# ydchen0806/CLC

Hardware: AMD Instinct MI355X
Metric: images/sec fwd+bwd @256x256 bs8; bpp+PSNR parity vs ref (higher is better)
Workload: dtype f32; 1 GPU; CLC N=64 lambda=0.0067 MSE, 256x256 bs8/GPU, n_refs=1: fwd + RD loss + bwd + clip_grad_norm + AdamW + aux step (configs[1]); global_batch=8, parallelism=dp1, ranks_seen=1, collective=none, hip_graph=True

## Files before the change

clc_amd/csrc/common.h:

```cpp
#pragma once
#include <hip/hip_runtime.h>
#include <stdarg.h>
#include <stdio.h>
#include "../../include/clc_hip.h"

typedef float f32x2 __attribute__((ext_vector_type(2)));
typedef float f32x4 __attribute__((ext_vector_type(4)));
typedef float f32x16 __attribute__((ext_vector_type(16)));

void clc_set_error(const char* fmt, ...);

enum {  CLC_TUNE_WGRAD_STREAMK = 1,
       CLC_TUNE_SPLITK_PIX = 4 , CLC_TUNE_SPLITK_MAXC = 5 ,
       CLC_TUNE_SPLITK_PF = 6 ,
       CLC_TUNE_1X1_TILE = 7 ,
       CLC_TUNE_XCD_MAP = 8 ,
       CLC_TUNE_WGRAD_DMA = 9 ,
       CLC_TUNE_REG_EPI = 10 ,
       CLC_TUNE_DGRAD_SPLITK = 11 ,
       CLC_TUNE_P1X1 = 13 ,
       CLC_TUNE_BF16 = 14 ,
       CLC_TUNE_TILE256 = 15 ,
       CLC_TUNE_ATTN_4B = 16 ,
       CLC_TUNE_HEAVY128 = 17 ,
       CLC_TUNE_ATTN_SPLIT = 18 ,
       CLC_TUNE_N16 = 20 ,
       CLC_TUNE_LIN = 21 ,
       CLC_TUNE_HALO = 22 ,
       CLC_TUNE_WINO = 23 ,
       CLC_TUNE_SPLIT = 24 ,
       CLC_TUNE_COUNT = 25 };
extern int clc_tuning[CLC_TUNE_COUNT];
int clc_conv_halo_launch(const void* conv_params, const float* wpk, hipStream_t st);
int clc_conv_wino_launch(const void* conv_params, const float* u, hipStream_t st);
int clc_conv5_launch(const clc_conv_desc* d, hipStream_t st);
size_t clc_conv5_wgrad_workspace_bytes(const clc_wgrad_desc* d);
int clc_conv5_wgrad_launch(const clc_wgrad_desc* d, hipStream_t st);
int clc_lin_launch(const float* x, int ldx, const float* w, const float* bias, const float* res, int ldr, float res_scale, float* y, int ldy, long M, int Cin,
                   int Cout, hipStream_t st);

#define CLC_CHECK(cond, ...)            \
  do {                                  \
    if (!(cond)) {                      \
      clc_set_error(__VA_ARGS__);       \
      return -1;                        \
    }                                   \
  } while (0)

#define CLC_LAUNCH_CHECK()                                              \
  do {                                                                  \
    hipError_t e_ = hipGetLastError();                                  \
    if (e_ != hipSuccess) {                                             \
      clc_set_error("%s:%d launch failed: %s", __FILE__, __LINE__, hipGetErrorString(e_)); \
      return -2;                                                        \
    }                                                                   \
  } while (0)

struct PerDeviceOnce {
  bool done[32] = {};
  bool first() {
    int d = 0;
    if (hipGetDevice(&d) != hipSuccess || d < 0 || d >= 32) return true;
    if (done[d]) return false;
    done[d] = true;
    return true;
  }
};
// ... 130 lines not shown
```

clc_amd/csrc/conv_igemm.hip:

```cpp
#include "common.h"
#ifndef CLC_PF32
#define CLC_PF32 3
#endif

namespace {
#include "conv_common.h"
template <int BM, int BN, int WM, int WN, bool TR>
__global__ __launch_bounds__(64 * WM * WN, (64 * WM * WN) >= 512 ? 4 : ((64 * WM * WN) >= 256 ? 2 : 4))
void conv_igemm_kernel(const ConvParams p) {
  constexpr int NT = 64 * WM * WN;
  constexpr int TM = BM / WM / 32, TN = BN / WN / 32;
  constexpr int A_P = BM * 8 / NT, B_P = BN * 8 / NT;
  static_assert(TM >= 1 && TN >= 1 && A_P * NT == BM * 8 && B_P * NT == BN * 8, "tile");
  extern __shared__ __attribute__((aligned(16))) float smem[];
  float* As = smem;
  float* Bs = smem + 2 * BM * LD;

  const int tid = threadIdx.x, lane = tid & 63, wave = tid >> 6;
  const int wm = wave / WN, wn = wave % WN;
  const int m0 = blockIdx.x * BM, n0 = blockIdx.y * BN;
  const int cls = blockIdx.z, ph = cls >> 1, pw = cls & 1;
  const bool half = p.transposed && p.stride == 2;
  const int DH = half ? p.OH / 2 : p.OH, DW = half ? p.OW / 2 : p.OW;
  const TapGrid tg = make_taps(p, ph, pw);
// ... 1020 lines not shown
extern "C" size_t clc_conv2d_workspace_bytes(const clc_conv_desc* d) {
  if (!d || d->ks == 5) return 0;
  ConvParams p;
  int classes = 1;
  if (fill_params(d, p, classes) < 0) return 0;
  const bool vec_ok = (d->Cin % 4 == 0) && (d->ldx % 4 == 0) && aligned16(d->x) && aligned16(d->w);
  if (!vec_ok || d->Cout < 64) return 0;
  const int img_pix = (d->transposed && d->stride == 2) ? (d->OH / 2) * (d->OW / 2) : d->OH * d->OW;
  if (img_pix > 1024) return 0;
  const int k = conv_ksplit(p, classes);
  return k > 1 ? (size_t)k * classes * p.M * p.Cout * sizeof(float) : 0;
}

extern "C" int clc_conv2d(const clc_conv_desc* d, clc_stream_t stream) {
  hipStream_t st = (hipStream_t)stream;
  if (d && d->ks == 5) return clc_conv5_launch(d, st);
  ConvParams p;
  int classes = 1;
  if (fill_params(d, p, classes) < 0) return -1;
  const bool vec_ok = (d->Cin % 4 == 0) && (d->ldx % 4 == 0) && aligned16(d->x) && aligned16(d->w);
  if (!vec_ok) {
    CLC_CHECK(!d->transposed && !d->xs, "clc_conv2d: unaligned/small-Cin path has no transposed / fused-activation mode (Cin=%d ldx=%d)", d->Cin, d->ldx);
    const int cgroups = (d->Cout + 3) / 4;
    const long total = (long)p.M * cgroups;
    hipLaunchKernelGGL(conv_direct_small_kernel, dim3((unsigned)((total + 255) / 256)), dim3(256), 0, st, p);
    CLC_LAUNCH_CHECK();
    return 1;
  }
  const int img_pix = (d->transposed && d->stride == 2) ? (d->OH / 2) * (d->OW / 2) : d->OH * d->OW;
  const int C = d->Cout;
  const int splitk_pix = clc_tuning[CLC_TUNE_SPLITK_PIX] > 0 ? clc_tuning[CLC_TUNE_SPLITK_PIX] : 256;
  const bool small_map = img_pix <= 256 || (img_pix <= splitk_pix && C <= clc_tuning[CLC_TUNE_SPLITK_MAXC]);
  if (small_map) {
    if (heavy128_split(p, classes) > 1) {
      use_split(p, d, classes);
      if (p.ksplit > 1) return launch<128, 128, 4, 2>(p, classes, st);
    }
    if (img_pix <= 256 && d->transposed && d->ks * d->ks * p.kc_tiles >= 60 && C >= 128 &&
        (long)((p.M + 63) / 64) * ((C + 63) / 64) * classes >= 128) {
      use_split(p, d, classes);
      return launch<64, 64, 2, 2>(p, classes, st);
    }
    const long wg32 = (long)((p.M + 31) / 32) * ((C + 31) / 32) * classes;
    if (C > 32 && wg32 > 256) return launch_splitk<64>(p, classes, st);
    return launch_splitk<32>(p, classes, st);
  }
  p.bf16 = clc_tuning[CLC_TUNE_BF16] != 0 && img_pix > 256;
  if ((clc_tuning[CLC_TUNE_WINO] & (d->transposed ? 2 : 1)) && d->w_wino && d->ks == 3 && d->stride == 1 && classes == 1) {
    const int v = clc_conv_wino_launch(&p, d->w_wino, st);
    if (v) return v;
  }
  if (clc_tuning[CLC_TUNE_HALO] && d->w_packed && d->ks == 3 && d->stride == 1 && classes == 1) {
    const int v = clc_conv_halo_launch(&p, d->w_packed, st);
    if (v) return v;
  }
  if (img_pix <= 1024) {
    if (C >= 64) {
      use_split(p, d, classes);
      return launch<64, 64, 2, 2>(p, classes, st);
    }
    return launch<64, 32, 2, 1>(p, classes, st);
  }
  if (clc_tuning[CLC_TUNE_LIN] && d->ks == 1 && d->stride == 1 && classes == 1 && vec_ok && !p.shuffle && !p.group_rows && !p.xs && p.in_op == CLC_IN_NONE &&
      p.act == CLC_ACT_NONE && p.norm == CLC_NORM_NONE && !p.y_pre && !p.res_gate && !p.out_gate && p.ldw == p.Cin && p.vec_epi && !p.bf16) {
    const int v = clc_lin_launch(p.x, p.ldx, p.w, p.bias, p.res, p.ldr, p.res_scale, p.y, p.ldy, p.M, p.Cin, p.Cout, st);
    if (v) { CLC_LAUNCH_CHECK(); return v; }
  }
  if (d->ks == 1 && C > 32 && vec_ok) {
    const int v = launch_p1x1(p, classes, st);
    if (v) return v;
  }
  if (clc_tuning[CLC_TUNE_1X1_TILE] && d->ks == 1 && p.kc_tiles <= clc_tuning[CLC_TUNE_1X1_TILE] && C > 32) return launch<128, 64, 4, 2>(p, classes, st);
  if (C % 128 == 0 || C >= 384) return launch<128, 128, 4, 2>(p, classes, st);
  if (clc_tuning[CLC_TUNE_TILE256] && d->ks == 3 && C > 32 && C <= 64 && p.M >= 256 * 512 && (!p.group_rows || p.group_rows % 256 == 0))
    return launch<256, 64, 4, 2>(p, classes, st);
  if (C > 32) return launch<128, 64, 4, 2>(p, classes, st);
  if (C <= 16 && vec_ok) {
    const int v = launch_n16(p, classes, st);
    if (v) return v;
  }
  if (clc_tuning[CLC_TUNE_TILE256] && d->ks == 3 && p.M % 128 == 0 && p.M >= 128 * 512) return launch<128, 32, 2, 1>(p, classes, st);
  return launch<64, 32, 2, 1>(p, classes, st);
// ... 10 lines not shown
```

clc_amd/csrc/conv_wino.hip:

```cpp
#include "common.h"

namespace {
#include "conv_common.h"

constexpr int TH = 8, TW = 16, HW = TW + 2, HPIX = (TH + 2) * HW;
constexpr int HALO_FLOATS = HPIX * 128;
constexpr int PIECES = HPIX / 2;

struct WinoParams {
  ConvParams c;
  const float* u;
  int items, ntn, ncg;
  unsigned u_bytes;
};

#ifndef WINO_AB
#define WINO_AB 0
#endif
#if WINO_AB & 32
__device__ unsigned long long wino_dbg[32];
#define WINO_STAMP(k) do { if (blockIdx.x == 0 && tid == 0 && it == i0 + 1) wino_dbg[k] = __builtin_amdgcn_s_memtime(); } while (0)
#else
#define WINO_STAMP(k) do { } while (0)
#endif
#define MFMA(a, b, c) __builtin_amdgcn_mfma_f32_32x32x2f32((a), (b), (c), 0, 0, 0)

constexpr int VB_FLOATS = 16 * 32 * 16;

template <bool SHUF>
__global__ __launch_bounds__(512, 1) void conv_wino_kernel(const WinoParams wp) {
  const ConvParams& p = wp.c;
  extern __shared__ __attribute__((aligned(16))) float smem[];
  float* halo = smem;
  float* bias_s = smem + HALO_FLOATS + 2 * VB_FLOATS;
  float* VV = smem + HALO_FLOATS;
  const int tid = threadIdx.x, lane = tid & 63, wave = tid >> 6;
  const int li = lane & 31, h = lane >> 5;
  const int tiles_w = p.W / TW, tiles_h = p.H / TH;
  const int KCT = wp.ncg * 4;
  const int NC16 = wp.ncg * 8;
  const int i0 = (int)((long)wp.items * blockIdx.x / gridDim.x), i1 = (int)((long)wp.items * (blockIdx.x + 1) / gridDim.x);
  const __amdgpu_buffer_rsrc_t xr = __builtin_amdgcn_make_buffer_rsrc(const_cast<float*>(p.x), 0, p.x_bytes, 0x00020000);
  const __amdgpu_buffer_rsrc_t ur = __builtin_amdgcn_make_buffer_rsrc(const_cast<float*>(wp.u), 0, wp.u_bytes, 0x00020000);
  const int q = tid & 3, t = (tid >> 2) & 31, part = tid >> 7;
  const int ty = t >> 3, tx = t & 7;
  const int wi = wave >> 1, nh = wave & 1;
// ... 204 lines not shown
        } else {
#pragma unroll 1
          for (int a = 0; a < 2; ++a)
#pragma unroll 1
            for (int e = 0; e < 4; ++e) {
              epilogue_store(p, a ? y[1][0][e] : y[0][0][e], bv[e], mrow0 + a * p.OW, co + e, p.OH, p.OW, 0, 0);
              epilogue_store(p, a ? y[1][1][e] : y[0][1][e], bv[e], mrow0 + a * p.OW + 1, co + e, p.OH, p.OW, 0, 0);
            }
        }
      }
      WINO_STAMP(15 + 3 * rd);
    }
  }
}

constexpr int HALO2_FLOATS = HPIX * 64;
constexpr int S2_FLOATS = 16 * 32 * 32;
constexpr int PIECES2 = HPIX / 4;
static_assert(HALO2_FLOATS <= S2_FLOATS, "the halo lies inside the output round's image");
__device__ __forceinline__ int wino64_swz(int hy, int hx) { return ((hx >> 1) & 3) | (((hy >> 1) & 3) << 2); }
__device__ __forceinline__ float add1(float a, float b) { float r; asm("v_add_f32 %0, %1, %2" : "=v"(r) : "v"(a), "v"(b)); return r; }
__device__ __forceinline__ float sub1(float a, float b) { float r; asm("v_sub_f32 %0, %1, %2" : "=v"(r) : "v"(a), "v"(b)); return r; }
__device__ __forceinline__ float fma1(float s, float b, float a) { float r; asm("v_fma_f32 %0, %1, %2, %3" : "=v"(r) : "s"(s), "v"(b), "v"(a)); return r; }

template <bool SHUF>
__global__ __launch_bounds__(256, 2) void conv_wino64_kernel(const WinoParams wp) {
  const ConvParams& p = wp.c;
  extern __shared__ __attribute__((aligned(16))) float smem[];
  float* halo = smem;
  float* S = smem;
  const int tid = threadIdx.x, lane = tid & 63, wave = __builtin_amdgcn_readfirstlane(tid >> 6);
  const int li = lane & 31, h = lane >> 5;
  const int tiles_w = p.W / TW, tiles_h = p.H / TH;
  const int KCT = wp.ncg * 2;
  const int NC16 = wp.ncg * 4;
  const int i0 = (int)((long)wp.items * blockIdx.x / gridDim.x), i1 = (int)((long)wp.items * (blockIdx.x + 1) / gridDim.x);
  const __amdgpu_buffer_rsrc_t xr = __builtin_amdgcn_make_buffer_rsrc(const_cast<float*>(p.x), 0, p.x_bytes, 0x00020000);
  const __amdgpu_buffer_rsrc_t ur = __builtin_amdgcn_make_buffer_rsrc(const_cast<float*>(wp.u), 0, wp.u_bytes, 0x00020000);
  const int ty = li >> 3, tx = li & 7;
  const int qo = tid & 15;
  const bool lean = epilogue_is_lean(p);
  const int ra = wave == 0 ? 0 : (wave == 2 ? 2 : 1), rb = wave == 0 ? 2 : (wave == 1 ? 2 : (wave == 2 ? 1 : 3));
  const float sg = wave == 1 ? 1.f : -1.f;
  int pa[2][2];
#pragma unroll
  for (int rr = 0; rr < 2; ++rr)
#pragma unroll
    for (int ch = 0; ch < 2; ++ch) {
      const int hy = 2 * ty + (rr ? rb : ra);
      pa[rr][ch] = (hy * HW + 2 * tx) * 256 + ((h ^ wino64_swz(hy, 2 * tx + 2 * ch)) << 4);
    }
  const char* hb = reinterpret_cast<const char*>(halo);
  auto read_row = [&](f32x4 (&d)[4], int rr, int kx) {
#pragma unroll
    for (int c = 0; c < 4; ++c) d[c] = *reinterpret_cast<const f32x4*>(hb + ((pa[rr][c >> 1] ^ kx) + c * 256));
  };
  const unsigned b_lane = (unsigned)lane * 16u;

  for (int it = i0; it < i1; ++it) {
    const int pt = it / wp.ntn, nt = it - pt * wp.ntn;
    const int txx = pt % tiles_w, t2 = pt / tiles_w, tyy = t2 % tiles_h, n = t2 / tiles_h;
    const int oy0 = tyy * TH, ox0 = txx * TW;
    f32x16 acc[4][2];
#pragma unroll
    for (int s = 0; s < 4; ++s)
#pragma unroll
      for (int nb = 0; nb < 2; ++nb)
#pragma unroll
        for (int r = 0; r < 16; ++r) acc[s][nb][r] = 0.f;
    f32x4 bq[4][2];
    auto load_b = [&](int s, int c16, int t8) {
      const int kcg = c16 >> 1, t8g = 2 * (c16 & 1) + t8;
#pragma unroll
      for (int nb = 0; nb < 2; ++nb)
        bq[s][nb] = buf_load4(ur, b_lane + (unsigned)((((((nt >> 1) * 16 + 4 * wave + s) * KCT + kcg) * 4 + 2 * (nt & 1) + nb) * 4 + t8g)) * 1024u);
    };
#pragma unroll
    for (int s = 0; s < 4; ++s) load_b(s, 0, 0);
    WINO_STAMP(0);

    for (int cg = 0; cg < wp.ncg; ++cg) {
      if (cg) __syncthreads();
      {
        const int org = ((n * p.H + oy0 - 1) * p.W + ox0 - 1) * p.ldx + cg * 64;
        int hy = 0, hx = 4 * wave + (lane >> 4);
#pragma unroll 1
        for (int pc = wave; pc < PIECES2; pc += 4) {
          const int iy = oy0 - 1 + hy, ix = ox0 - 1 + hx;
          const bool ok = (unsigned)iy < (unsigned)p.H && (unsigned)ix < (unsigned)p.W;
          const int c = (lane & 15) ^ wino64_swz(hy, hx);
          dma16(xr, halo + pc * 256, ok ? (unsigned)(org + (hy * p.W + hx) * p.ldx + c * 4) * 4u : kOOB);
          hx += 16;
          if (hx >= HW) { hx -= HW; ++hy; }
        }
        asm volatile("s_waitcnt vmcnt(0)" ::: "memory");
      }
      __syncthreads();
      WINO_STAMP(1);
      f32x4 aq[2][4];
      f32x4 da[4], db[4];
      auto rows_T = [&]() {
#pragma unroll
        for (int c = 0; c < 4; ++c)
#pragma unroll
          for (int e = 0; e < 4; ++e) da[c][e] = fma1(sg, db[c][e], da[c][e]);
      };
      auto cols_B = [&](f32x4 (&v)[4]) {
#pragma unroll
        for (int e = 0; e < 4; ++e) {
          v[0][e] = sub1(da[0][e], da[2][e]);
          v[1][e] = add1(da[1][e], da[2][e]);
          v[2][e] = sub1(da[2][e], da[1][e]);
          v[3][e] = sub1(da[1][e], da[3][e]);
        }
      };
      read_row(da, 0, 0);
      read_row(db, 1, 0);
      rows_T();
      cols_B(aq[0]);
      WINO_STAMP(2);
#pragma unroll 1
      for (int kc = 0; kc < 4; ++kc) {
        if (cg == 0) WINO_STAMP(3 + kc);
        const int c16 = cg * 4 + kc;
#pragma unroll
        for (int t8 = 0; t8 < 2; ++t8) {
          const int kxn = t8 == 0 ? (4 * kc + 2) << 4 : (4 * ((kc + 1) & 3)) << 4;
          const int c16n = t8 == 0 ? c16 : (c16 + 1 < NC16 ? c16 + 1 : 0);
#pragma unroll
          for (int s = 0; s < 4; ++s) {
            if (s == 0) read_row(da, 0, kxn);
            else if (s == 1) read_row(db, 1, kxn);
            else if (s == 2) rows_T();
            else cols_B(aq[t8 ^ 1]);
            __builtin_amdgcn_sched_barrier(0);
#pragma unroll
            for (int ss = 0; ss < 4; ++ss)
#pragma unroll
              for (int nb = 0; nb < 2; ++nb) acc[s][nb] = MFMA(aq[t8][s][ss], bq[s][nb][ss], acc[s][nb]);
            load_b(s, c16n, t8 ^ 1);
            __builtin_amdgcn_sched_barrier(0);
          }
        }
      }
    }
    WINO_STAMP(11);
    {
      const int co = nt * 64 + (qo >> 3) * 32 + (qo & 7) * 4;
      const f32x4 bv = epilogue_bias4(p.bias, co);
      __syncthreads();
      WINO_STAMP(13);
#pragma unroll
      for (int b = 0; b < 2; ++b) {
        float* dst = S + ((wave * 2 + b) * 32) * 64;
#pragma unroll
// ... 100 lines not shown
    f32x4 u[4];
    u[0] = tt[i][0];
    u[1] = 0.5f * ((tt[i][0] + tt[i][1]) + tt[i][2]);
    u[2] = 0.5f * ((tt[i][0] - tt[i][1]) + tt[i][2]);
    u[3] = tt[i][2];
#pragma unroll
    for (int j = 0; j < 4; ++j) {
      const size_t idx = ((((((size_t)nt * 16 + (i * 4 + j)) * KCT + kcg) * 4 + nb) * 4 + t8) * 64 + lane);
      *reinterpret_cast<f32x4*>(out + idx * 4) = u[j];
    }
  }
}
__global__ void filter_wino_kernel(const float* __restrict__ w, float* __restrict__ out, int N, int K, int flip) {
  const long e = (long)blockIdx.x * blockDim.x + threadIdx.x;
  if (e >= (long)N * K / 4) return;
  wino_u_one(w, out, e, K, flip);
}
__global__ void filter_wino_batched_kernel(const clc_wino_entry* __restrict__ table, int n_entries) {
  int lo = 0, hi = n_entries - 1;
  const int b = blockIdx.x;
  while (lo < hi) {
    const int mid = (lo + hi + 1) >> 1;
    if (table[mid].block_begin <= b) lo = mid; else hi = mid - 1;
  }
  const clc_wino_entry en = table[lo];
  const long e = (long)(b - en.block_begin) * blockDim.x + threadIdx.x;
  if (e >= (long)en.N * en.K / 4) return;
  wino_u_one(en.w, en.out, e, en.K, en.flip);
}

}

extern "C" int clc_filter_wino(const float* w, float* out, int N, int K, int flip, clc_stream_t stream) {
  CLC_CHECK(w && out && N > 0 && N % 64 == 0 && K > 0 && K % 64 == 0 && aligned16(w) && aligned16(out),
            "clc_filter_wino: rows and channels must be positive multiples of 64, pointers 16-B aligned (got N=%d K=%d)", N, K);
  const long total = (long)N * K / 4;
  hipLaunchKernelGGL(filter_wino_kernel, dim3((unsigned)((total + 255) / 256)), dim3(256), 0, (hipStream_t)stream, w, out, N, K, flip);
  CLC_LAUNCH_CHECK();
  return 0;
}
extern "C" int clc_filter_wino_batched(const clc_wino_entry* table_dev, int n_entries, int total_blocks, clc_stream_t stream) {
  CLC_CHECK(table_dev && n_entries > 0 && total_blocks > 0, "clc_filter_wino_batched: bad args");
  hipLaunchKernelGGL(filter_wino_batched_kernel, dim3(total_blocks), dim3(256), 0, (hipStream_t)stream, table_dev, n_entries);
  CLC_LAUNCH_CHECK();
  return 0;
}

int clc_conv_wino_launch(const void* conv_params, const float* u, hipStream_t st) {
  const ConvParams& p = *reinterpret_cast<const ConvParams*>(conv_params);
  if (!u || p.ks != 3 || p.stride != 1 || p.pad != 1 || p.Cin % 64 || p.Cin > 1024 || p.Cout % 64 || p.H % TH || p.W % TW || p.OH != p.H || p.OW != p.W) return 0;
  if (p.xs || p.in_op != CLC_IN_NONE || p.group_rows || p.bf16 || p.ksplit > 1 || p.ldx % 4 || !aligned16(p.x) || !aligned16(u)) return 0;
  const bool shuf = p.shuffle != 0;
  if (!shuf && !p.vec_epi) return 0;
  const size_t ub = (size_t)((p.Cout + 127) / 128 * 128) * 16 * p.Cin * 4;
  if (ub >= (1ull << 31)) return 0;
  const int mode = clc_tuning[CLC_TUNE_WINO];
  const int ptiles = p.N * (p.H / TH) * (p.W / TW);
  const bool can128 = p.Cin % 128 == 0 && p.Cout % 128 == 0 && !(mode & 8);
  const bool wide = can128 && ptiles * (p.Cout / 128) >= 192;
  if (!wide && (!(mode & 4) || ptiles * (p.Cout / 64) < 128)) return 0;
  const int nw = wide ? 128 : 64;
  WinoParams wp;
  wp.c = p;
  wp.u = u;
  wp.ntn = p.Cout / nw;
  wp.ncg = p.Cin / nw;
  wp.items = ptiles * wp.ntn;
  wp.u_bytes = (unsigned)ub;
  static PerDeviceOnce once[2];
  const int k = shuf ? 1 : 0;
  if (wide) {
    const int grid = wp.items < 256 ? wp.items : 256;
    const int lds = (HALO_FLOATS + 2 * VB_FLOATS + 128) * 4;
    static PerDeviceOnce oncep[2];
    if (shuf) {
      if (oncep[0].first()) (void)hipFuncSetAttribute(reinterpret_cast<const void*>(conv_wino_kernel<true>), hipFuncAttributeMaxDynamicSharedMemorySize, lds);
      hipLaunchKernelGGL(conv_wino_kernel<true>, dim3(grid), dim3(512), lds, st, wp);
    } else {
      if (oncep[1].first()) (void)hipFuncSetAttribute(reinterpret_cast<const void*>(conv_wino_kernel<false>), hipFuncAttributeMaxDynamicSharedMemorySize, lds);
      hipLaunchKernelGGL(conv_wino_kernel<false>, dim3(grid), dim3(512), lds, st, wp);
    }
  } else {
    const int grid = wp.items < 512 ? wp.items : 512;
    const int lds = S2_FLOATS * 4;
    if (shuf) {
      if (once[k].first()) (void)hipFuncSetAttribute(reinterpret_cast<const void*>(conv_wino64_kernel<true>), hipFuncAttributeMaxDynamicSharedMemorySize, lds);
      hipLaunchKernelGGL(conv_wino64_kernel<true>, dim3(grid), dim3(256), lds, st, wp);
    } else {
      if (once[k].first()) (void)hipFuncSetAttribute(reinterpret_cast<const void*>(conv_wino64_kernel<false>), hipFuncAttributeMaxDynamicSharedMemorySize, lds);
      hipLaunchKernelGGL(conv_wino64_kernel<false>, dim3(grid), dim3(256), lds, st, wp);
    }
  }
  CLC_LAUNCH_CHECK();
  return (13 << 20) | ((wide ? 0 : 1) << 12) | (wp.ncg << 4) | ((p.transposed ? 1 : 0) << 1) | (shuf ? 1 : 0);
}

#if WINO_AB & 32
extern "C" int clc_wino_debug(unsigned long long* out_host) {
  return (int)hipMemcpyFromSymbol(out_host, HIP_SYMBOL(wino_dbg), sizeof(unsigned long long) * 32);
}
#endif
// ... 1 lines not shown
```

clc_amd/lib.py:

```python
from __future__ import annotations

import ctypes as C
import os

_HERE = os.path.dirname(os.path.abspath(__file__))
LIB_PATH = os.environ.get("CLC_LIB_PATH") or os.path.join(_HERE, "libclc_hip.so")

ACT_NONE, ACT_LRELU, ACT_RELU, ACT_GELU, ACT_HALFTANH, ACT_SIGMOID, ACT_SAVED_DERIV = 0, 1, 2, 3, 4, 5, 6
IN_NONE, IN_SQUARE = 0, 1
NORM_NONE, NORM_GDN, NORM_IGDN, NORM_MUL2 = 0, 1, 2, 3
AR_SRC_DENSE, AR_SRC_PIXEL, AR_SRC_TAPS = 0, 1, 2
AR_ENCODE, AR_DECODE = 0, 1
GMM_R = 32
GMM_ROW_STRIDE = 2 * GMM_R + 3

fp = C.c_void_p


class ConvDesc(C.Structure):
    _fields_ = [("x", fp), ("N", C.c_int), ("H", C.c_int), ("W", C.c_int), ("Cin", C.c_int), ("ldx", C.c_int),
                ("w", fp), ("bias", fp),
                ("y", fp), ("OH", C.c_int), ("OW", C.c_int), ("Cout", C.c_int), ("ldy", C.c_int),
                ("ks", C.c_int), ("stride", C.c_int), ("pad", C.c_int),
                ("transposed", C.c_int), ("in_op", C.c_int), ("act", C.c_int),
                ("norm", C.c_int), ("mul", fp), ("ldm", C.c_int),
                ("res", fp), ("ldr", C.c_int), ("res_scale", C.c_float),
                ("y_pre", fp), ("ldp", C.c_int),
                ("shuffle", C.c_int), ("res_first", C.c_int),
                ("xs", fp), ("ldxs", C.c_int), ("xs_act", C.c_int), ("xs_pre", C.c_int),
                ("w2", fp), ("bias2", fp), ("pre_deriv", C.c_int),
                ("res_gate", fp), ("ldg", C.c_int), ("res_gate_act", C.c_int), ("res_gate_pre", C.c_int),
                ("out_gate", fp), ("ldog", C.c_int), ("out_gate_act", C.c_int), ("out_gate_pre", C.c_int),
                ("w3", fp), ("bias3", fp), ("w4", fp), ("bias4", fp),
                ("workspace", fp), ("workspace_bytes", C.c_size_t), ("batch_variant_ok", C.c_int), ("w_packed", fp), ("w_wino", fp)]


class WgradDesc(C.Structure):
    _fields_ = [("x", fp), ("N", C.c_int), ("H", C.c_int), ("W", C.c_int), ("Cin", C.c_int), ("ldx", C.c_int),
                ("dy", fp), ("OH", C.c_int), ("OW", C.c_int), ("Cout", C.c_int), ("lddy", C.c_int),
                ("dw", fp), ("dbias", fp),
                ("ks", C.c_int), ("stride", C.c_int), ("pad", C.c_int),
                ("in_op", C.c_int), ("accumulate", C.c_int),
                ("workspace", fp), ("workspace_bytes", C.c_size_t),
                ("dys", fp), ("lddys", C.c_int), ("dys_act", C.c_int), ("dys_pre", C.c_int)]


class RUDesc(C.Structure):
    _fields_ = [("x", fp), ("ldx", C.c_int), ("t1", fp), ("t2", fp), ("y", fp),
                ("N", C.c_int), ("H", C.c_int), ("W", C.c_int), ("C", C.c_int), ("sets", C.c_int),
                ("w1", fp * 4), ("b1", fp * 4), ("w2", fp * 4), ("b2", fp * 4), ("w3", fp * 4), ("b3", fp * 4),
                ("saved_y", fp), ("saved_t2", fp), ("saved_t1", fp)]


class MlpDesc(C.Structure):
    _fields_ = [("x", fp), ("ldx", C.c_int), ("w1", fp), ("b1", fp), ("w2", fp), ("b2", fp), ("res", fp), ("ldr", C.c_int),
                ("y", fp), ("ldy", C.c_int), ("M", C.c_long), ("Cin", C.c_int), ("Chid", C.c_int), ("Cout", C.c_int),
                ("dy", fp), ("lddy", C.c_int), ("w2t", fp), ("dx", fp), ("lddx", C.c_int), ("dh", fp), ("g", fp), ("h", fp),
                ("ln_gamma", fp), ("ln_beta", fp), ("ln_out", fp), ("ln_ws", fp)]


class LnLinDesc(C.Structure):
    _fields_ = [("x", fp), ("ldx", C.c_int), ("ln_gamma", fp), ("ln_beta", fp), ("w", fp), ("b", fp), ("y", fp), ("ln_out", fp),
                ("M", C.c_long), ("Cin", C.c_int), ("Cout", C.c_int), ("dy", fp), ("wt", fp), ("dx", fp), ("lddx", C.c_int),
                ("dadd", fp), ("ldadd", C.c_int), ("ln_ws", fp)]


class GDNEntry(C.Structure):
# ... 303 lines not shown
```

clc_amd/ops.py:

```python
from __future__ import annotations

import contextlib
import ctypes as C
import functools
import math

import torch
from torch.autograd import Function

from . import lib as _lib
from .lib import (ACT_GELU, ACT_HALFTANH, ACT_LRELU, ACT_NONE, ACT_RELU, ACT_SAVED_DERIV, ACT_SIGMOID, IN_NONE, IN_SQUARE, NORM_GDN,
                  NORM_IGDN, NORM_MUL2, NORM_NONE)

CL = torch.channels_last

WGRAD_DEFER = False


class _DeviceState:

    __slots__ = ("pending", "pending_flop", "pending_streams", "pending_post", "last_defer_vid", "pending_reduce", "keepalive",
                 "group_ws")

    def __init__(self):
# ... 387 lines not shown
def note_use(w, kind):
    if USES is not None:
        USES.add((id(w), kind))


def halo_ok(N, H, W, Cin, rows, ks, stride):
    if not (ks == 3 and stride == 1 and Cin in (128, 64) and rows % Cin == 0 and H % 8 == 0 and W % 16 == 0):
        return 0
    if not (_L().clc_get_tuning(22) & (1 if Cin == 128 else 2)):
        return 0
    return Cin if N * (H // 8) * (W // 16) * (rows // Cin) >= 128 else 0


def halo_pack(wk, rows, K=128):
    out = torch.empty(rows * 9 * K, device=wk.device, dtype=torch.float32)
    _lib.check(_L().clc_filter_pack_halo(wk.data_ptr(), out.data_ptr(), int(rows), int(K), _stream()), "clc_filter_pack_halo")
    return out


def halo_packed(w, transposed_image=None):
    tr = transposed_image is not None
    kind = "halo_t" if tr else "halo"
    note_use(w, kind)
    pk = _image(w, kind)
    if pk is not None:
        return pk
    if tr:
        return halo_pack(transposed_image, transposed_image.shape[0], w.shape[0])
    return halo_pack(to_kernel_weight(w), w.shape[0], w.shape[1])




def wino_ok(N, H, W, Cin, rows, ks, stride, transposed=False):
    mode = _L().clc_get_tuning(23)
    if not (mode & (2 if transposed else 1)) or not (ks == 3 and stride == 1 and H % 8 == 0 and W % 16 == 0 and Cin <= 1024):
        return False
    ptiles = N * (H // 8) * (W // 16)
    if Cin % 128 == 0 and rows % 128 == 0 and not (mode & 8) and ptiles * (rows // 128) >= 192:
        return True
    return bool(mode & 4) and Cin % 64 == 0 and rows % 64 == 0 and ptiles * (rows // 64) >= 128


def wino_pack(wk, rows, K, flip=False):
    out = torch.empty(-(-rows // 128) * 128 * 16 * K, device=wk.device, dtype=torch.float32)
    _lib.check(_L().clc_filter_wino(wk.data_ptr(), out.data_ptr(), int(rows), int(K), int(bool(flip)), _stream()), "clc_filter_wino")
    return out


def wino_packed(w, transposed_image=None):
    tr = transposed_image is not None
    kind = "wino_t" if tr else "wino"
    note_use(w, kind)
    u = _image(w, kind)
    if u is not None:
        return u
    if tr:
        return wino_pack(transposed_image, transposed_image.shape[0], w.shape[0], flip=True)
    return wino_pack(to_kernel_weight(w), w.shape[0], w.shape[1])


def conv_raw(x, w, bias=None, *, ks, stride=1, pad=None, act=ACT_NONE, in_op=IN_NONE, norm=NORM_NONE, mul=None,
             res=None, res_scale=1.0, res_first=False, y_pre=None, shuffle=False, transposed=False, out=None, out_hw=None,
             xs=None, xs_act=ACT_NONE, xs_pre=False, w2=None, bias2=None, pre_deriv=False, res_gate=None, out_gate=None, wx=None, batch_variant_ok=False,
             wpk=None, wwino=None):
    _require_gpu(x, "conv2d")
    x, xp, N, H, W, Cin, ldx = nhwc(x)
    Cout = w.shape[0]
    pad = ks // 2 if pad is None else pad
    if transposed:
        OH, OW = out_hw
    else:
        OH, OW = (H + 2 * pad - ks) // stride + 1, (W + 2 * pad - ks) // stride + 1
    if out is None:
        out = new_act(N, Cout // 4, 2 * OH, 2 * OW, x) if shuffle else new_act(N, Cout, OH, OW, x)
    o, op, _, _, _, _, ldy = nhwc(out)
    assert o is out, "conv2d: output buffer must be pixel-major"
    d = _lib.ConvDesc()
    d.x, d.N, d.H, d.W, d.Cin, d.ldx = xp, N, H, W, Cin, ldx
    d.w = w.data_ptr()
    d.bias = bias.data_ptr() if bias is not None else None
    d.y, d.OH, d.OW, d.Cout, d.ldy = op, OH, OW, Cout, ldy
    d.ks, d.stride, d.pad = ks, stride, pad
    d.transposed, d.in_op, d.act, d.norm, d.shuffle = int(transposed), in_op, act, norm, int(shuffle)
    keep = [x, w, bias, out]
    if w2 is not None:
        d.w2 = w2.data_ptr()
        d.bias2 = bias2.data_ptr() if bias2 is not None else None
        if wx is not None:
            (w3, b3), (w4, b4) = wx
            d.w3, d.w4 = w3.data_ptr(), w4.data_ptr()
            d.bias3 = b3.data_ptr() if b3 is not None else None
            d.bias4 = b4.data_ptr() if b4 is not None else None
            keep += [w3, b3, w4, b4]
    if mul is not None:
        m, mp, *_r, ldm = nhwc(mul)
        d.mul, d.ldm = mp, ldm
        keep.append(m)
    if res is not None:
        r, rp, *_r, ldr = nhwc(res)
        d.res, d.ldr, d.res_scale, d.res_first = rp, ldr, float(res_scale), int(res_first)
        keep.append(r)
        if res_gate is not None:
            gt, gp, *_r, ldg = nhwc(res_gate[0])
            d.res_gate, d.ldg, d.res_gate_act, d.res_gate_pre = gp, ldg, int(res_gate[1]), int(res_gate[2])
            keep.append(gt)
    if out_gate is not None:
        ot, otp, *_r, ldog = nhwc(out_gate[0])
        d.out_gate, d.ldog, d.out_gate_act, d.out_gate_pre = otp, ldog, int(out_gate[1]), int(out_gate[2])
        keep.append(ot)
    if y_pre is not None:
        q, qp, *_r, ldp = nhwc(y_pre)
        assert q is y_pre
        d.y_pre, d.ldp = qp, ldp
        d.pre_deriv = int(pre_deriv)
    if xs is not None:
        xs_t, xsp, *_r, ldxs = nhwc(xs)
        d.xs, d.ldxs, d.xs_act, d.xs_pre = xsp, ldxs, xs_act, int(xs_pre)
        keep.append(xs_t)
    d.batch_variant_ok = int(bool(batch_variant_ok))
    if wpk is not None:
        d.w_packed = wpk.data_ptr()
        keep.append(wpk)
    if wwino is not None:
        d.w_wino = wwino.data_ptr()
        keep.append(wwino)
    if (transposed and H * W <= 1024) or (batch_variant_ok and ks == 3 and OH * OW <= 256):
        nws = _lib.load().clc_conv2d_workspace_bytes(C.byref(d))
        if nws:
            ws = torch.empty((nws + 3) // 4, device=x.device, dtype=torch.float32)
            d.workspace, d.workspace_bytes = ws.data_ptr(), nws
            keep.append(ws)
    if PROFILE is None:
        _lib.check(_lib.load().clc_conv2d(C.byref(d), _stream()), "clc_conv2d")
    else:
        e0, e1 = torch.cuda.Event(enable_timing=True), torch.cuda.Event(enable_timing=True)
        e0.record()
        variant = _lib.check(_lib.load().clc_conv2d(C.byref(d), _stream()), "clc_conv2d")
        e1.record()
        pix = N * H * W if transposed else N * OH * OW
        opix = N * OH * OW
        nbytes = 4.0 * (N * H * W * Cin + Cout * ks * ks * Cin
                        + opix * Cout * (1 + (res is not None) + (mul is not None) + (y_pre is not None) + (out_gate is not None)))
        PROFILE.append(ProfRec("conv_igemm" if variant != 1 else "conv_direct_small", variant, 2.0 * pix * ks * ks * Cin * Cout, e0, e1,
                               f"{'dgrad' if transposed else 'fwd'} {Cin}->{Cout} k{ks} s{stride} {N}x{H}x{W}" + (" +actbwd" if xs is not None else "") + (" +sq" if in_op == IN_SQUARE else "")
                               + "".join(t for t, on in ((" b", bias is not None), (f" a{act}", act != ACT_NONE), (" res", res is not None), (" mul", mul is not None),
                                                         (" pre", y_pre is not None), (" rg", res_gate is not None), (" og", out_gate is not None), (" w2", w2 is not None and wx is None), (" w4", wx is not None)) if on),
                               nbytes, relaunch=(lambda d=d, keep=keep: _lib.load().clc_conv2d(C.byref(d), _stream()))))
    return out


def im2col_small(x, ks, stride, ldc=32):
    _require_gpu(x, "im2col_small")
    assert not x.requires_grad
    x, xp, N, H, W, Cc, ldx = nhwc(x)
    pad = ks // 2
    OH, OW = (H + 2 * pad - ks) // stride + 1, (W + 2 * pad - ks) // stride + 1
    col = new_act(N, ldc, OH, OW, x)
    _lib.check(_L().clc_im2col_small(xp, ldx, N, H, W, Cc, ks, stride, pad, col.data_ptr(), ldc, OH, OW, _stream()), "clc_im2col_small")
# ... 220 lines not shown
            dz = torch.nn.functional.pixel_unshuffle(dz, 2).contiguous(memory_format=CL)
        dx = dw = db = dw2 = db2 = None
        w3, b3, w4, b4 = ctx.quad
        dwq = [None] * 4
        pad = ks // 2
        if need_w or need_b:
            if w3 is not None:
                q = x.shape[0] // 4
                res4 = []
                for k, (wk_, bk_) in enumerate(((w, ctx.bias_ref), (w2, b2), (w3, b3), (w4, b4))):
                    sl = slice(k * q, (k + 1) * q)
                    fwk = dict(dys=saved_act[sl], dys_act=act, dys_pre=ctx.use_pre) if fuse else {}
                    res4.append(_ConvFn._wgrad(x[sl], dz[sl], wk_, bk_, has_b, need_w, need_b, ks, stride, pad, fwk))
                (dw, db), (dw2, db2) = res4[0], res4[1]
                dwq = [res4[2][0], res4[2][1], res4[3][0], res4[3][1]]
            elif w2 is None:
                fw = dict(dys=saved_act, dys_act=act, dys_pre=ctx.use_pre) if fuse else {}
                dw, db = _ConvFn._wgrad(x, dz, w, ctx.bias_ref, has_b, need_w, need_b, ks, stride, pad, fw)
            else:
                h = x.shape[0] // 2
                fw1 = dict(dys=saved_act[:h], dys_act=act, dys_pre=ctx.use_pre) if fuse else {}
                fw2 = dict(dys=saved_act[h:], dys_act=act, dys_pre=ctx.use_pre) if fuse else {}
                dw, db = _ConvFn._wgrad(x[:h], dz[:h], w, ctx.bias_ref, has_b, need_w, need_b, ks, stride, pad, fw1)
                dw2, db2 = _ConvFn._wgrad(x[h:], dz[h:], w2, b2, has_b, need_w, need_b, ks, stride, pad, fw2)
        if need_x:
            extra, extra_scale, gate = fold_in.take() if fold_in is not None else (None, 1.0, None)
            gs = ctx.grad_slot
            dx_out = gs[0].view(x, gs[1], gs[2], x.shape[1]) if gs is not None else None
            og = None
            if gate_in is not None and gate_in.saved is not None and extra is None and ctx.park_dx is None:
                og = (gate_in.saved, gate_in.act, gate_in.pre)
                gate_in.done = True
            wt1 = _wt_of(w)
            wwino = (wino_packed(w, wt1) if (w2 is None and not fa and wino_ok(dz.shape[0], dz.shape[2], dz.shape[3], Cout, Cin, ks, stride, transposed=True)) else None)
            wpk = (halo_packed(w, wt1) if (wwino is None and w2 is None and not fa and halo_ok(dz.shape[0], dz.shape[2], dz.shape[3], Cout, Cin, ks, stride)) else None)
            dx = conv_raw(dz, wt1, None, ks=ks, stride=stride, pad=pad, transposed=True, out_hw=(x.shape[2], x.shape[3]),
                          w2=(_wt_of(w2) if w2 is not None else None), wx=(((_wt_of(w3), None), (_wt_of(w4), None)) if w3 is not None else None),
                          res=extra, res_scale=extra_scale, res_gate=gate, out=dx_out, out_gate=og, wpk=wpk, wwino=wwino, **fa)
        elif fold_in is not None:
            fold_in.consumed = True
        if dx is not None and ctx.park_dx is not None and ctx.park_dx.park(dx):
            dx = None
        return (dx, dw, db, dres, None, None, None, None, None, None, dw2, db2, None, None, None, None, None, None, None) + tuple(dwq)


def conv2d(x, w, b=None, *, stride=1, act=ACT_NONE, res=None, res_scale=1.0, shuffle=False, res_first=False, w2=None, b2=None,
           fold_in=None, fold_out=None, out=None, grad_slot=None, park_dx=None, gate_in=None, gate_out=None, wx=None):
    ks = w.shape[2] if w.dim() == 4 else 1
    (w3, b3), (w4, b4) = wx if wx is not None else ((None, None), (None, None))
    _note_grad_mode()
    return _ConvFn.apply(x, w, b, res, ks, stride, act, float(res_scale), bool(shuffle), bool(res_first), w2, b2, fold_in, fold_out, out,
                         grad_slot, park_dx, gate_in, gate_out, w3, b3, w4, b4)


def colsum(x):
    x, xp, N, H, W, Cc, ld = nhwc(x)
    nb = _L().clc_colsum_workspace_bytes(N * H * W, Cc)
    ws = torch.empty((nb + 3) // 4, device=x.device, dtype=torch.float32)
    out = torch.empty(Cc, device=x.device, dtype=torch.float32)
    _lib.check(_L().clc_colsum(xp, ld, N * H * W, Cc, out.data_ptr(), 0, ws.data_ptr(), nb, _stream()), "clc_colsum")
    return out


def patch_filter(wk, ldc):
    rows = wk.shape[0]
    m = wk.permute(0, 2, 3, 1).reshape(rows, -1)
    return torch.nn.functional.pad(m, (0, ldc - m.shape[1]))


class _ConvTranspose5Fn(Function):

# ... 2100 lines not shown
```

include/clc_hip.h:

```cpp
#ifndef CLC_HIP_H
#define CLC_HIP_H
#include <stddef.h>
#include <stdint.h>

#ifdef __cplusplus
extern "C" {
#endif

typedef void* clc_stream_t;

const char* clc_last_error(void);
int clc_version(void);
int clc_set_tuning(int key, int value);
int clc_get_tuning(int key);
int clc_kernel_config_tag(void);
unsigned clc_kernel_config_hash(void);

enum { CLC_ACT_NONE = 0, CLC_ACT_LRELU = 1, CLC_ACT_RELU = 2, CLC_ACT_GELU = 3, CLC_ACT_HALFTANH = 4 ,
       CLC_ACT_SIGMOID = 5 ,
       CLC_ACT_SAVED_DERIV = 6  };
enum { CLC_IN_NONE = 0, CLC_IN_SQUARE = 1 };
enum { CLC_NORM_NONE = 0, CLC_NORM_GDN = 1, CLC_NORM_IGDN = 2,
       CLC_NORM_MUL2 = 3  };

typedef struct {
  const float* x; int N, H, W, Cin, ldx;
  const float* w;
  const float* bias;
  float* y; int OH, OW, Cout, ldy;
  int ks, stride, pad;
  int transposed;
  int in_op;
  int act;
  int norm; const float* mul; int ldm;
  const float* res; int ldr; float res_scale;
  float* y_pre; int ldp;
  int shuffle;
  int res_first;
  const float* xs; int ldxs; int xs_act; int xs_pre;
  const float* w2; const float* bias2;
  int pre_deriv;
  const float* res_gate; int ldg; int res_gate_act; int res_gate_pre;
  const float* out_gate; int ldog; int out_gate_act; int out_gate_pre;
  const float* w3; const float* bias3; const float* w4; const float* bias4;
  void* workspace; size_t workspace_bytes;
  int batch_variant_ok;
  const float* w_packed;
  const float* w_wino;
} clc_conv_desc;

int clc_conv2d(const clc_conv_desc* d, clc_stream_t stream);
int clc_filter_pack_halo(const float* w, float* out, int N, int K, clc_stream_t stream);
typedef struct { const float* w; float* out; int N, K, block_begin; } clc_halo_pack_entry;
int clc_filter_pack_halo_batched(const clc_halo_pack_entry* table_dev, int n_entries, int total_blocks, clc_stream_t stream);
int clc_filter_wino(const float* w, float* out, int N, int K, int flip, clc_stream_t stream);
typedef struct { const float* w; float* out; int N, K, flip, block_begin; } clc_wino_entry;
int clc_filter_wino_batched(const clc_wino_entry* table_dev, int n_entries, int total_blocks, clc_stream_t stream);
size_t clc_conv2d_workspace_bytes(const clc_conv_desc* d);

typedef struct {
  const float* x; int N, H, W, Cin, ldx;
  const float* dy; int OH, OW, Cout, lddy;
  float* dw; float* dbias;
  int ks, stride, pad;
  int in_op;
  int accumulate;
  void* workspace; size_t workspace_bytes;
  const float* dys; int lddys; int dys_act; int dys_pre;
} clc_wgrad_desc;

size_t clc_conv2d_wgrad_workspace_bytes(const clc_wgrad_desc* d);
int clc_conv2d_wgrad(const clc_wgrad_desc* d, clc_stream_t stream);
int clc_conv2d_wgrad_batched(const clc_wgrad_desc* descs, int count, clc_stream_t stream);
size_t clc_conv2d_wgrad_group_workspace_bytes(void);
size_t clc_conv2d_wgrad_sk_workspace_bytes(const clc_wgrad_desc* d);
int clc_conv2d_wgrad_variant(const clc_wgrad_desc* d);
int clc_conv2d_wgrad_batched_sk(const clc_wgrad_desc* descs, int count, void* group_workspace, size_t group_workspace_bytes,
                                clc_stream_t stream);

int clc_filter_transpose(const float* w, float* wt, int Cout, int T, int Cin, clc_stream_t stream);
typedef struct { const float* w; float* wt; int Cout, T, Cin, tile_begin; } clc_transpose_entry;
// ... 408 lines not shown
```

Before: 335.8 images/sec.

## Route small-map transposed 3x3 dgrad convs through Winograd, including two-weight-set batches

Adds a small-feature-map path (<=256 pixels) that sends transposed 3x3 stride-1 data-gradient convolutions to the Winograd kernel, which now also supports Cin that is a multiple of 32 and a second weight set selected per batch half (u2, for grouped rows). The kernel gains per-item weight-resource selection, channel-tail masking in the halo load and a variable inner-loop trip count. The Python side packs Winograd filters for the second weight too and gates eligibility with a tile-count floor. This aims to cut direct-conv cost on small late-stage maps, at the risk of low occupancy on small grids and extra filter-transform launches.

```diff
diff --git a/clc_amd/csrc/common.h b/clc_amd/csrc/common.h
--- a/clc_amd/csrc/common.h
+++ b/clc_amd/csrc/common.h
@@ -32,7 +32,7 @@
        CLC_TUNE_COUNT = 25 };
 extern int clc_tuning[CLC_TUNE_COUNT];
 int clc_conv_halo_launch(const void* conv_params, const float* wpk, hipStream_t st);
-int clc_conv_wino_launch(const void* conv_params, const float* u, hipStream_t st);
+int clc_conv_wino_launch(const void* conv_params, const float* u, const float* u2, hipStream_t st);
 int clc_conv5_launch(const clc_conv_desc* d, hipStream_t st);
 size_t clc_conv5_wgrad_workspace_bytes(const clc_wgrad_desc* d);
 int clc_conv5_wgrad_launch(const clc_wgrad_desc* d, hipStream_t st);
diff --git a/clc_amd/csrc/conv_igemm.hip b/clc_amd/csrc/conv_igemm.hip
--- a/clc_amd/csrc/conv_igemm.hip
+++ b/clc_amd/csrc/conv_igemm.hip
@@ -1076,6 +1076,11 @@
   const int splitk_pix = clc_tuning[CLC_TUNE_SPLITK_PIX] > 0 ? clc_tuning[CLC_TUNE_SPLITK_PIX] : 256;
   const bool small_map = img_pix <= 256 || (img_pix <= splitk_pix && C <= clc_tuning[CLC_TUNE_SPLITK_MAXC]);
   if (small_map) {
+    if (img_pix <= 256 && d->transposed && !(clc_tuning[CLC_TUNE_WINO] & 16) && d->w_wino && (!d->w2 || d->w_wino2) && !d->w3 && d->ks == 3 &&
+        d->stride == 1 && classes == 1) {
+      const int v = clc_conv_wino_launch(&p, d->w_wino, d->w2 ? d->w_wino2 : nullptr, st);
+      if (v) return v;
+    }
     if (heavy128_split(p, classes) > 1) {
       use_split(p, d, classes);
       if (p.ksplit > 1) return launch<128, 128, 4, 2>(p, classes, st);
@@ -1091,7 +1096,7 @@
   }
   p.bf16 = clc_tuning[CLC_TUNE_BF16] != 0 && img_pix > 256;
   if ((clc_tuning[CLC_TUNE_WINO] & (d->transposed ? 2 : 1)) && d->w_wino && d->ks == 3 && d->stride == 1 && classes == 1) {
-    const int v = clc_conv_wino_launch(&p, d->w_wino, st);
+    const int v = clc_conv_wino_launch(&p, d->w_wino, nullptr, st);
     if (v) return v;
   }
   if (clc_tuning[CLC_TUNE_HALO] && d->w_packed && d->ks == 3 && d->stride == 1 && classes == 1) {
diff --git a/clc_amd/csrc/conv_wino.hip b/clc_amd/csrc/conv_wino.hip
--- a/clc_amd/csrc/conv_wino.hip
+++ b/clc_amd/csrc/conv_wino.hip
@@ -12,6 +12,8 @@
   const float* u;
   int items, ntn, ncg;
   unsigned u_bytes;
+  int nc16, set_n;
+  const float* u2;
 };
 
 #ifndef WINO_AB
@@ -282,11 +284,10 @@
   const int tid = threadIdx.x, lane = tid & 63, wave = __builtin_amdgcn_readfirstlane(tid >> 6);
   const int li = lane & 31, h = lane >> 5;
   const int tiles_w = p.W / TW, tiles_h = p.H / TH;
-  const int KCT = wp.ncg * 2;
-  const int NC16 = wp.ncg * 4;
+  const int NC16 = wp.nc16;
+  const int KCT = NC16 >> 1;
   const int i0 = (int)((long)wp.items * blockIdx.x / gridDim.x), i1 = (int)((long)wp.items * (blockIdx.x + 1) / gridDim.x);
   const __amdgpu_buffer_rsrc_t xr = __builtin_amdgcn_make_buffer_rsrc(const_cast<float*>(p.x), 0, p.x_bytes, 0x00020000);
-  const __amdgpu_buffer_rsrc_t ur = __builtin_amdgcn_make_buffer_rsrc(const_cast<float*>(wp.u), 0, wp.u_bytes, 0x00020000);
   const int ty = li >> 3, tx = li & 7;
   const int qo = tid & 15;
   const bool lean = epilogue_is_lean(p);
@@ -311,6 +312,7 @@
     const int pt = it / wp.ntn, nt = it - pt * wp.ntn;
     const int txx = pt % tiles_w, t2 = pt / tiles_w, tyy = t2 % tiles_h, n = t2 / tiles_h;
     const int oy0 = tyy * TH, ox0 = txx * TW;
+    const __amdgpu_buffer_rsrc_t ur = __builtin_amdgcn_make_buffer_rsrc(const_cast<float*>(wp.u2 != nullptr && n >= wp.set_n ? wp.u2 : wp.u), 0, wp.u_bytes, 0x00020000);
     f32x16 acc[4][2];
 #pragma unroll
     for (int s = 0; s < 4; ++s)
@@ -333,12 +335,13 @@
       if (cg) __syncthreads();
       {
         const int org = ((n * p.H + oy0 - 1) * p.W + ox0 - 1) * p.ldx + cg * 64;
+        const int cleft = (p.Cin - cg * 64) >> 2;
         int hy = 0, hx = 4 * wave + (lane >> 4);
 #pragma unroll 1
         for (int pc = wave; pc < PIECES2; pc += 4) {
           const int iy = oy0 - 1 + hy, ix = ox0 - 1 + hx;
-          const bool ok = (unsigned)iy < (unsigned)p.H && (unsigned)ix < (unsigned)p.W;
           const int c = (lane & 15) ^ wino64_swz(hy, hx);
+          const bool ok = (unsigned)iy < (unsigned)p.H && (unsigned)ix < (unsigned)p.W && c < cleft;
           dma16(xr, halo + pc * 256, ok ? (unsigned)(org + (hy * p.W + hx) * p.ldx + c * 4) * 4u : kOOB);
           hx += 16;
           if (hx >= HW) { hx -= HW; ++hy; }
@@ -369,8 +372,9 @@
       rows_T();
       cols_B(aq[0]);
       WINO_STAMP(2);
-#pragma unroll 1
-      for (int kc = 0; kc < 4; ++kc) {
+      const int nkc = NC16 - cg * 4 < 4 ? NC16 - cg * 4 : 4;
+#pragma unroll 1
+      for (int kc = 0; kc < nkc; ++kc) {
         if (cg == 0) WINO_STAMP(3 + kc);
         const int c16 = cg * 4 + kc;
 #pragma unroll
@@ -537,8 +541,8 @@
 }
 
 extern "C" int clc_filter_wino(const float* w, float* out, int N, int K, int flip, clc_stream_t stream) {
-  CLC_CHECK(w && out && N > 0 && N % 64 == 0 && K > 0 && K % 64 == 0 && aligned16(w) && aligned16(out),
-            "clc_filter_wino: rows and channels must be positive multiples of 64, pointers 16-B aligned (got N=%d K=%d)", N, K);
+  CLC_CHECK(w && out && N > 0 && N % 64 == 0 && K > 0 && K % 32 == 0 && aligned16(w) && aligned16(out),
+            "clc_filter_wino: rows must be a positive multiple of 64, channels of 32, pointers 16-B aligned (got N=%d K=%d)", N, K);
   const long total = (long)N * K / 4;
   hipLaunchKernelGGL(filter_wino_kernel, dim3((unsigned)((total + 255) / 256)), dim3(256), 0, (hipStream_t)stream, w, out, N, K, flip);
   CLC_LAUNCH_CHECK();
@@ -551,27 +555,43 @@
   return 0;
 }
 
-int clc_conv_wino_launch(const void* conv_params, const float* u, hipStream_t st) {
+constexpr int kSmallMapFloor = 112;
+int clc_conv_wino_launch(const void* conv_params, const float* u, const float* u2, hipStream_t st) {
   const ConvParams& p = *reinterpret_cast<const ConvParams*>(conv_params);
-  if (!u || p.ks != 3 || p.stride != 1 || p.pad != 1 || p.Cin % 64 || p.Cin > 1024 || p.Cout % 64 || p.H % TH || p.W % TW || p.OH != p.H || p.OW != p.W) return 0;
-  if (p.xs || p.in_op != CLC_IN_NONE || p.group_rows || p.bf16 || p.ksplit > 1 || p.ldx % 4 || !aligned16(p.x) || !aligned16(u)) return 0;
+  const int mode = clc_tuning[CLC_TUNE_WINO];
+  const bool small = p.H * p.W <= 256;
+  if (!u || p.ks != 3 || p.stride != 1 || p.pad != 1 || p.Cin % 32 || p.Cin > 1024 || p.Cout % 64 || p.H % TH || p.W % TW || p.OH != p.H || p.OW != p.W) return 0;
+  if (p.xs || p.in_op != CLC_IN_NONE || p.bf16 || p.ksplit > 1 || p.ldx % 4 || !aligned16(p.x) || !aligned16(u)) return 0;
+  if (small) {
+    if (!p.transposed || (mode & 16)) return 0;
+    if (p.group_rows && (!u2 || !aligned16(u2) || p.w3 || p.bias || p.N % 2 || p.group_rows != (p.N / 2) * p.H * p.W)) return 0;
+  } else if (p.Cin % 64 || p.group_rows) {
+    return 0;
+  }
   const bool shuf = p.shuffle != 0;
   if (!shuf && !p.vec_epi) return 0;
   const size_t ub = (size_t)((p.Cout + 127) / 128 * 128) * 16 * p.Cin * 4;
   if (ub >= (1ull << 31)) return 0;
-  const int mode = clc_tuning[CLC_TUNE_WINO];
   const int ptiles = p.N * (p.H / TH) * (p.W / TW);
   const bool can128 = p.Cin % 128 == 0 && p.Cout % 128 == 0 && !(mode & 8);
-  const bool wide = can128 && ptiles * (p.Cout / 128) >= 192;
-  if (!wide && (!(mode & 4) || ptiles * (p.Cout / 64) < 128)) return 0;
+  const bool wide = !small && can128 && ptiles * (p.Cout / 128) >= 192;
+  if (small) {
+    const int floor = (mode >> 8) & 0xFFFF;
+    if (ptiles * (p.Cout / 64) < (floor ? floor : kSmallMapFloor)) return 0;
+  } else if (!wide && (!(mode & 4) || ptiles * (p.Cout / 64) < 128)) {
+    return 0;
+  }
   const int nw = wide ? 128 : 64;
   WinoParams wp;
   wp.c = p;
   wp.u = u;
   wp.ntn = p.Cout / nw;
-  wp.ncg = p.Cin / nw;
+  wp.ncg = (p.Cin + nw - 1) / nw;
   wp.items = ptiles * wp.ntn;
   wp.u_bytes = (unsigned)ub;
+  wp.nc16 = p.Cin / 16;
+  wp.set_n = p.N / 2;
+  wp.u2 = p.group_rows ? u2 : nullptr;
   static PerDeviceOnce once[2];
   const int k = shuf ? 1 : 0;
   if (wide) {
diff --git a/clc_amd/lib.py b/clc_amd/lib.py
--- a/clc_amd/lib.py
+++ b/clc_amd/lib.py
@@ -32,7 +32,8 @@
                 ("res_gate", fp), ("ldg", C.c_int), ("res_gate_act", C.c_int), ("res_gate_pre", C.c_int),
                 ("out_gate", fp), ("ldog", C.c_int), ("out_gate_act", C.c_int), ("out_gate_pre", C.c_int),
                 ("w3", fp), ("bias3", fp), ("w4", fp), ("bias4", fp),
-                ("workspace", fp), ("workspace_bytes", C.c_size_t), ("batch_variant_ok", C.c_int), ("w_packed", fp), ("w_wino", fp)]
+                ("workspace", fp), ("workspace_bytes", C.c_size_t), ("batch_variant_ok", C.c_int), ("w_packed", fp), ("w_wino", fp),
+                ("w_wino2", fp)]
 
 
 class WgradDesc(C.Structure):
diff --git a/clc_amd/ops.py b/clc_amd/ops.py
--- a/clc_amd/ops.py
+++ b/clc_amd/ops.py
@@ -443,8 +443,16 @@
 
 
 
-def wino_ok(N, H, W, Cin, rows, ks, stride, transposed=False):
+WINO_SMALL_MAP_FLOOR = 112
+
+
+def wino_ok(N, H, W, Cin, rows, ks, stride, transposed=False, sets=1):
     mode = _L().clc_get_tuning(23)
+    if ks == 3 and stride == 1 and H % 8 == 0 and W % 16 == 0 and Cin <= 1024 and H * W <= 256 and transposed and not (mode & 16) and sets <= 2:
+        if Cin % 32 == 0 and rows % 64 == 0 and N % sets == 0 and N * (H // 8) * (W // 16) * (rows // 64) >= (((mode >> 8) & 0xFFFF) or WINO_SMALL_MAP_FLOOR):
+            return True
+    if sets != 1:
+        return False
     if not (mode & (2 if transposed else 1)) or not (ks == 3 and stride == 1 and H % 8 == 0 and W % 16 == 0 and Cin <= 1024):
         return False
     ptiles = N * (H // 8) * (W // 16)
@@ -474,7 +482,7 @@
 def conv_raw(x, w, bias=None, *, ks, stride=1, pad=None, act=ACT_NONE, in_op=IN_NONE, norm=NORM_NONE, mul=None,
              res=None, res_scale=1.0, res_first=False, y_pre=None, shuffle=False, transposed=False, out=None, out_hw=None,
              xs=None, xs_act=ACT_NONE, xs_pre=False, w2=None, bias2=None, pre_deriv=False, res_gate=None, out_gate=None, wx=None, batch_variant_ok=False,
-             wpk=None, wwino=None):
+             wpk=None, wwino=None, wwino2=None):
     _require_gpu(x, "conv2d")
     x, xp, N, H, W, Cin, ldx = nhwc(x)
     Cout = w.shape[0]
@@ -536,6 +544,9 @@
     if wwino is not None:
         d.w_wino = wwino.data_ptr()
         keep.append(wwino)
+        if wwino2 is not None and w2 is not None:
+            d.w_wino2 = wwino2.data_ptr()
+            keep.append(wwino2)
     if (transposed and H * W <= 1024) or (batch_variant_ok and ks == 3 and OH * OW <= 256):
         nws = _lib.load().clc_conv2d_workspace_bytes(C.byref(d))
         if nws:
@@ -822,11 +833,14 @@
                 og = (gate_in.saved, gate_in.act, gate_in.pre)
                 gate_in.done = True
             wt1 = _wt_of(w)
-            wwino = (wino_packed(w, wt1) if (w2 is None and not fa and wino_ok(dz.shape[0], dz.shape[2], dz.shape[3], Cout, Cin, ks, stride, transposed=True)) else None)
+            wok = not fa and wino_ok(dz.shape[0], dz.shape[2], dz.shape[3], Cout, Cin, ks, stride, transposed=True,
+                                     sets=4 if w3 is not None else (2 if w2 is not None else 1))
+            wwino = wino_packed(w, wt1) if wok else None
+            wwino2 = wino_packed(w2, _wt_of(w2)) if (wok and w2 is not None) else None
             wpk = (halo_packed(w, wt1) if (wwino is None and w2 is None and not fa and halo_ok(dz.shape[0], dz.shape[2], dz.shape[3], Cout, Cin, ks, stride)) else None)
             dx = conv_raw(dz, wt1, None, ks=ks, stride=stride, pad=pad, transposed=True, out_hw=(x.shape[2], x.shape[3]),
                           w2=(_wt_of(w2) if w2 is not None else None), wx=(((_wt_of(w3), None), (_wt_of(w4), None)) if w3 is not None else None),
-                          res=extra, res_scale=extra_scale, res_gate=gate, out=dx_out, out_gate=og, wpk=wpk, wwino=wwino, **fa)
+                          res=extra, res_scale=extra_scale, res_gate=gate, out=dx_out, out_gate=og, wpk=wpk, wwino=wwino, wwino2=wwino2, **fa)
         elif fold_in is not None:
             fold_in.consumed = True
         if dx is not None and ctx.park_dx is not None and ctx.park_dx.park(dx):
diff --git a/include/clc_hip.h b/include/clc_hip.h
--- a/include/clc_hip.h
+++ b/include/clc_hip.h
@@ -47,6 +47,7 @@
   int batch_variant_ok;
   const float* w_packed;
   const float* w_wino;
+  const float* w_wino2;
 } clc_conv_desc;
 
 int clc_conv2d(const clc_conv_desc* d, clc_stream_t stream);
```

Result: no change. 338.4 images/sec, median of 6 (+0.8%).
